# oarodriguez/PhD-QMCLib

Measured on AMD Instinct MI355X. Metric: walker-steps/sec, higher is better.
Workload: dtype f64

## Files before the change

### phd_qmclib_amd/csrc/qmc_device.h

```cpp
#pragma once

#include <hip/hip_runtime.h>
#include <stdint.h>

#include "qmc_math.h"

#define QMC_PI 3.141592653589793238462643383279502884

#define QMC_NSEC 32
#define QMC_SEC_COPIES 1024
#define QMC_NDIAG 4
#if defined(QMC_TIMING)
#define QMC_SECTION(name) qmc_stamp(m, qmc_sec_id(name))
#define QMC_SECTION_PHASE(off) qmc_stamp_phase(off)
#elif defined(QMC_CUTS)
#define QMC_SECTION(name)                                                     \
    do {                                                                      \
        if (m.sec_cut == qmc_sec_id(name) + QMC_SEC_OFF)                      \
            __builtin_amdgcn_endpgm();                                        \
    } while (0)
#define QMC_SECTION_PHASE(off) do { } while (0)
#elif defined(QMC_SECTIONS)
#define QMC_SECTION(name) asm volatile("; SECTION " name)
#define QMC_SECTION_PHASE(off) do { } while (0)
// ... 135 lines not shown
                                                uint32_t stream, double &u0,
                                                double &u1)
{
    uint32_t c[4] = { slot, step, index, stream };
    philox4x32_10(c, (uint32_t)seed, (uint32_t)(seed >> 32));
    u0 = u53(c[0], c[1]);
    u1 = u53(c[2], c[3]);
}

__device__ __forceinline__ void philox2x32_10(uint32_t &c0, uint32_t &c1,
                                              uint32_t k)
{
#pragma unroll
    for (int r = 0; r < 10; ++r) {
        const uint64_t p = (uint64_t)0xD256D193u * c0;
        const uint32_t n0 = (uint32_t)(p >> 32) ^ k ^ c1;
        c1 = (uint32_t)p;
        c0 = n0;
        k += 0x9E3779B9u;
    }
}

__device__ __forceinline__ void vmc_move_block(uint64_t seed, uint32_t slot,
                                               uint32_t step, uint32_t index,
                                               uint32_t &w0, uint32_t &w1)
{
    uint32_t key = (uint32_t)seed ^ ((uint32_t)(seed >> 32) * 0x85EBCA6Bu);
    key += (step >> 26) * 0x632BE5ABu + (slot >> 28) * 0xC2B2AE35u;
    w0 = ((step & 0x3FFFFFFu) << 6) | ((slot >> 22) & 0x3Fu);
    w1 = ((slot & 0x3FFFFFu) << 10) | (index & 0x3FFu);
    philox2x32_10(w0, w1, key);
}

__device__ __forceinline__ double vmc_move_unit(uint32_t w0)
{
    return fma((double)w0, 0x1p-32, 0x1p-33 - 0.5);
}

__device__ __forceinline__ void normal2_from_uniforms(double u0, double u1,
                                                      double &g0, double &g1)
{
    double r = fast_sqrt(fmax(-2.0 * log_pos(1.0 - u0), 1e-300));
    double s, c;
    sincos_halfpi(4.0 * u1, s, c);
    g0 = r * c;
    g1 = r * s;
}

__device__ __forceinline__ void philox_normal2(uint64_t seed, uint32_t slot,
                                               uint32_t step, uint32_t index,
                                               uint32_t stream, double &g0,
                                               double &g1)
{
    double u0, u1;
    philox_uniform2(seed, slot, step, index, stream, u0, u1);
    normal2_from_uniforms(u0, u1, g0, g1);
}

__device__ __forceinline__ void normal2_from_words(uint32_t w0, uint32_t w1,
                                                   double &g0, double &g1)
{
    const double u0 = fma((double)w0, 0x1p-32, 0x1p-33);
    const double u1 = fma((double)w1, 0x1p-32, 0x1p-33);
    const double r = fast_sqrt(-2.0 * log_pos(u0));
    double s, c;
    sincos_halfpi(4.0 * u1, s, c);
    g0 = r * c;
    g1 = r * s;
}

__device__ __forceinline__ void dmc_normal2(uint64_t seed, uint32_t slot,
                                            uint32_t step2, uint32_t index,
                                            double &g0, double &g1)
{
    uint32_t key = (uint32_t)seed ^ ((uint32_t)(seed >> 32) * 0x85EBCA6Bu);
    key += 0x27D4EB2Fu;
    key += (step2 >> 26) * 0x632BE5ABu + (slot >> 28) * 0xC2B2AE35u;
    uint32_t w0 = ((step2 & 0x3FFFFFFu) << 6) | ((slot >> 22) & 0x3Fu);
    uint32_t w1 = ((slot & 0x3FFFFFu) << 10) | (index & 0x3FFu);
    philox2x32_10(w0, w1, key);
    normal2_from_words(w0, w1, g0, g1);
}

__device__ __forceinline__ double wrap_box(double z, double L)
{
    double zw = (z < 0.0) ? z + L : (z >= L) ? z - L : z;
    const bool far = z < -L || z >= 2.0 * L;
    if (__builtin_expect(__ballot(far) != 0ull, 0)) {
        const double r = fma(-L, floor(z / L), z);
        zw = far ? (r < 0.0 ? r + L : r) : zw;
    }
    return zw;
}

template <int G, int P>
struct SlotMap {
    static constexpr bool CONSECUTIVE = (G == 64) && (P >= 2);
};

template <int G, bool PAD>
__device__ __forceinline__ int lanes_in_use(const DevModel &m)
{
    return PAD ? m.ge : G;
}

template <int G, int P, bool PAD>
__device__ __forceinline__ int walker_n(const DevModel &m)
{
    return PAD ? m.n : G * P;
}

template <int G, int P, bool PAD>
__device__ __forceinline__ int lane_particle(const DevModel &m, int gl, int p)
{
    if (SlotMap<G, P>::CONSECUTIVE) return P * gl + p;
    if (!PAD) return gl + G * p;
    const int ge = m.ge;
    return gl < ge ? gl + ge * p : m.n;
}

template <int N>
__device__ __forceinline__ double row_ror_f64(double v)
{
    const int lo = __builtin_amdgcn_update_dpp(0, __double2loint(v), 0x120 + N,
                                               0xf, 0xf, false);
    const int hi = __builtin_amdgcn_update_dpp(0, __double2hiint(v), 0x120 + N,
                                               0xf, 0xf, false);
    return __hiloint2double(hi, lo);
}

template <int G>
__device__ __forceinline__ double group_sum(double v)
{
    static_assert(G >= 16, "lane groups are 16, 32 or 64 lanes");
    v += row_ror_f64<8>(v);
    v += row_ror_f64<4>(v);
    v += row_ror_f64<2>(v);
    v += row_ror_f64<1>(v);
#pragma unroll
    for (int m = 16; m < G; m <<= 1)
        v += __shfl_xor(v, m, 64);
    return v;
}

__device__ __forceinline__ double wave_sum_mfma(double v)
{
    const double r = __builtin_amdgcn_mfma_f64_4x4x4f64(v, 1.0, 0.0, 0, 0, 0);
    double t = __builtin_amdgcn_mfma_f64_4x4x4f64(r, 1.0, 0.0, 0, 0, 0);
    t += row_ror_f64<4>(t);
    t += row_ror_f64<8>(t);
    return t;
}

template <int G, int P>
__device__ __forceinline__ void resort_step(double (&z)[P], int (&lab)[P],
                                            int gl, unsigned parity, int n,
                                            double L, double half_L,
                                            int ge = G)
{
    const int lane = threadIdx.x & 63, base = lane - gl;
    int pg = (parity & 1u) ? ((gl & 1) ? gl + 1 : gl - 1) : (gl ^ 1);
    const bool wrap_hi = pg >= ge, wrap_lo = pg < 0;
    if (wrap_hi) pg = 0;
    if (wrap_lo) pg = ge - 1;
    double z0[P]; int l0[P];
#pragma unroll
    for (int a = 0; a < P; ++a) { z0[a] = z[a]; l0[a] = lab[a]; }
#pragma unroll
    for (int a = 0; a < P; ++a) {
        const int want = wrap_hi ? (a + 1) % P : (wrap_lo ? (a + P - 1) % P : a);
        double zp = 0.0; int lp = 0;
#pragma unroll
        for (int b = 0; b < P; ++b) {
            double zz = __shfl(z0[b], base + pg, 64);
            int ll = __shfl(l0[b], base + pg, 64);
            if (b == want) { zp = zz; lp = ll; }
        }
        const bool valid = gl < ge && (gl + ge * a) < n &&
                           (pg + ge * want) < n;
        const bool lower = wrap_hi ? true : (wrap_lo ? false : gl < pg);
        double d = lower ? zp - z0[a] : z0[a] - zp;
        if (d > half_L) d -= L;
        if (d < -half_L) d += L;
        if (valid && d < 0.0) { z[a] = zp; lab[a] = lp; }
    }
}

template <int G>
__device__ __forceinline__ void resort_linear(double &z, int &lab, int gl,
                                              unsigned parity, int ge)
{
    const int lane = threadIdx.x & 63, base = lane - gl;
    const int pg = (parity & 1u) ? ((gl & 1) ? gl + 1 : gl - 1) : (gl ^ 1);
    const bool has = gl < ge && pg >= 0 && pg < ge;
    const int src = base + (has ? pg : gl);
    const double zp = __shfl(z, src, 64);
    const int lp = __shfl(lab, src, 64);
    const bool take = has && ((gl < pg) ? zp < z : zp > z);
    if (take) { z = zp; lab = lp; }
}

template <int G>
__device__ __forceinline__ int group_ror1_b32(int x)
{
    static_assert(G == 64 || G == 16, "a DPP rotation exists for 16 and 64 lanes");
    if (G == 64) return __builtin_amdgcn_update_dpp(x, x, 0x13C, 0xf, 0xf, false);
    return __builtin_amdgcn_update_dpp(x, x, 0x121, 0xf, 0xf, false);
}
template <int G>
__device__ __forceinline__ double group_ror1(double v)
{
    return __hiloint2double(group_ror1_b32<G>(__double2hiint(v)),
                            group_ror1_b32<G>(__double2loint(v)));
}
template <int G>
__device__ __forceinline__ float group_ror1(float v)
{
    return __int_as_float(group_ror1_b32<G>(__float_as_int(v)));
}

__device__ __forceinline__ double readlane_f64(double v, int lane)
{
    const int lo = __builtin_amdgcn_readlane(__double2loint(v), lane);
    const int hi = __builtin_amdgcn_readlane(__double2hiint(v), lane);
    return __hiloint2double(hi, lo);
}

__device__ __forceinline__ void anchor_seam(double &z, int &lab,
                                            int ge )
{
    const int lane = threadIdx.x & 63;
    const double z0 = readlane_f64(z, 0), zl = readlane_f64(z, ge - 1);
    if (zl < z0) {
        const double z1 = readlane_f64(z, 1), zl1 = readlane_f64(z, ge - 2);
        int src = lane;
        if (zl < z1) {
            if (lane < ge) src = lane == 0 ? ge - 1 : lane - 1;
        } else if (z0 > zl1) {
            if (lane < ge) src = lane == ge - 1 ? 0 : lane + 1;
        }
        z = __shfl(z, src, 64);
        lab = __shfl(lab, src, 64);
    }
}

template <int P>
__device__ __forceinline__ void order_pair(double &za, int &la, double &zb,
                                           int &lb, bool valid)
{
    const bool sw = valid && zb < za;
    const double t = za; const int u = la;
    za = sw ? zb : za; la = sw ? lb : la;
    zb = sw ? t : zb; lb = sw ? u : lb;
}

template <int P>
__device__ __forceinline__ void resort_linear_rows(double (&z)[P], int (&lab)[P],
                                                   int gl, unsigned parity, int n)
{
    static_assert(P % 2 == 0, "consecutive slots: an even number per lane");
    const int i0 = P * gl;
    if (!(parity & 1u)) {
#pragma unroll
        for (int a = 0; a + 1 < P; a += 2)
            order_pair<P>(z[a], lab[a], z[a + 1], lab[a + 1], i0 + a + 1 < n);
    } else {
        const int lane = threadIdx.x & 63;
        const double up = __shfl(z[0], lane + 1, 64);
        const int lup = __shfl(lab[0], lane + 1, 64);
        const double dn = __shfl(z[P - 1], lane - 1, 64);
        const int ldn = __shfl(lab[P - 1], lane - 1, 64);
        const double top = z[P - 1], bot = z[0];
#pragma unroll
        for (int a = 1; a + 1 < P; a += 2)
            order_pair<P>(z[a], lab[a], z[a + 1], lab[a + 1], i0 + a + 1 < n);
        if (gl < 63 && i0 + P < n && up < top) { z[P - 1] = up; lab[P - 1] = lup; }
        if (gl > 0 && i0 < n && dn > bot) { z[0] = dn; lab[0] = ldn; }
    }
}

template <int P, typename T>
__device__ __forceinline__ T row_reg(const T (&v)[P], int r)
{
    T x = v[0];
#pragma unroll
    for (int a = 1; a < P; ++a) x = (r == a) ? v[a] : x;
    return x;
}

template <int P>
__device__ __forceinline__ void anchor_seam_rows(double (&z)[P], int (&lab)[P],
                                                 int n)
{
    const int lane = threadIdx.x & 63;
    const int ln = (n - 1) / P, rn = (n - 1) % P;
    const double z0 = readlane_f64(z[0], 0);
    const double zl = readlane_f64(row_reg<P>(z, rn), ln);
    if (zl < z0) {
        const double z1 = readlane_f64(z[1], 0);
        const int ln2 = (n - 2) / P, rn2 = (n - 2) % P;
        const double zl1 = readlane_f64(row_reg<P>(z, rn2), ln2);
        if (zl < z1) {
            const int labl = __builtin_amdgcn_readlane(row_reg<P>(lab, rn), ln);
            double zin = __shfl(z[P - 1], lane - 1, 64);
            int lin = __shfl(lab[P - 1], lane - 1, 64);
            if (lane == 0) { zin = zl; lin = labl; }
#pragma unroll
            for (int a = P - 1; a >= 1; --a) { z[a] = z[a - 1]; lab[a] = lab[a - 1]; }
// ... 906 lines not shown
```

### phd_qmclib_amd/csrc/qmc_kernels.h

```cpp
#pragma once

#include "qmc_device.h"
#include "qmc_sorted64.h"
#include "qmc_sorted128.h"

static constexpr int BLOCK = 256;

static constexpr int BLOCK64 = 64;
template <int G>
struct WalkBlock {
    static constexpr int N = (G == 64) ? BLOCK64 : BLOCK;
};

template <int GPB>
__device__ __forceinline__ long long walker_of_block(unsigned b, int grp)
{
    if (GPB == 1)
        return ((long long)(b >> 7) << 7) + ((b & 7u) << 4) + ((b & 127u) >> 3);
    return (long long)b * GPB + grp;
}

template <int G, int P, bool PAD, bool ZC, bool DMC = false>
struct StepLds {
    static constexpr int NROWS =
// ... 147 lines not shown
struct alignas(64) VmcRec {
    double wf;
    double ecarry;
    double sum_e, sum_e2;
    long long n_acc;
    long long spare[3];
};
static_assert(sizeof(VmcRec) == 64, "one record = 8 eight-byte words");
typedef unsigned int VmcRecWords __attribute__((ext_vector_type(16)));
#define QMC_CONST __attribute__((address_space(4)))
__device__ __forceinline__ double vmc_rec_word(const VmcRecWords &r, int k)
{
    return __hiloint2double((int)r[2 * k + 1], (int)r[2 * k]);
}

struct VmcArgs {
    double *pos;
    unsigned short *label;
    VmcRec *rec;
    double *ser_wf, *ser_e;
    unsigned char *ser_stat;
    double *ser_pos;
    const double *tape;
    long long tape_steps;
    long long tape_idx;
    long long W;
    long long y;
    unsigned int nsteps;
    int forced;
    int reset_sums;
    int gaussian;
    unsigned int step;
    unsigned int chain0;
    unsigned long long seed;
    double move_spread;
};

template <int G, int P, bool ZC>
struct VmcFused {
    static constexpr bool ON = G == 64 && !ZC && (P == 1 || P == 2);
};

template <int G, int P, bool PAD, bool ZC, bool LEAN, typename R = double,
          bool STEADY = false>
__global__ void __launch_bounds__(WalkBlock<G>::N, lb_waves(G, P, ZC, LB_VMC_P2))
vmc_step_kernel(const DevModel *__restrict__ mp, VmcArgs a)
{
    static_assert(LEAN || !STEADY, "the steady variant is a LEAN kernel");
    const DevModel &m = *mp;
    [[maybe_unused]] constexpr int QMC_SEC_OFF = 0;
    QMC_SECTION("top");
    extern __shared__ double smem[];
    constexpr int GPB = WalkBlock<G>::N / G;
    const int grp = threadIdx.x / G, gl = threadIdx.x % G;
    static_assert(StepLds<G, P, PAD, ZC>::DOUBLES >= GroupLds<G, P, ZC>::DOUBLES,
                  "eval_walker is the fallback on the same LDS region");
    double *lds = smem + (size_t)grp * StepLds<G, P, PAD, ZC>::DOUBLES;
    const long long w = walker_of_block<GPB>(blockIdx.x, grp);
    const bool active = w < a.W;
    if (GPB == 1 && !active) return;
    const long long wr = active ? w : 0;
    const int n = walker_n<G, P, PAD>(m);
    const unsigned int slot = a.chain0 + (unsigned int)wr;
    const bool forced = !STEADY && a.forced != 0;
    const bool reset_sums = !STEADY && a.reset_sums != 0;

    const long long wl = (G == 64) ? qmc_uniform(wr) : wr;
    double wf_cur, e_cur, se = 0.0, se2 = 0.0;
    long long na = 0;
    if constexpr (G == 64) {
        const VmcRecWords r = *(const QMC_CONST VmcRecWords *)(a.rec + wl);
        wf_cur = vmc_rec_word(r, 0);
        e_cur = vmc_rec_word(r, 1);
        se = vmc_rec_word(r, 2);
        se2 = vmc_rec_word(r, 3);
        na = __double_as_longlong(vmc_rec_word(r, 4));
        if (reset_sums) { se = 0.0; se2 = 0.0; na = 0; }
    } else {
        wf_cur = a.rec[wl].wf;
        e_cur = a.rec[wl].ecarry;
    }

    constexpr bool FUSED = STEADY && VmcFused<G, P, ZC>::ON;
    double zc[P];
    int labc[P];
    [[maybe_unused]] double thr = 0.0;
    if constexpr (FUSED) {
#pragma unroll
        for (int p = 0; p < P; ++p) {
            int i = lane_particle<G, P, PAD>(m, gl, p);
            zc[p] = (i < n) ? a.pos[wr * n + i] : 0.0;
            labc[p] = (i < n) ? (int)a.label[wr * n + i] : i;
        }
    }
    bool any_acc = false;
    const unsigned int nst = FUSED ? a.nsteps : 1u;
    bool acc = false;
    [[maybe_unused]] const int gl_top = gl;
    for (unsigned int s = 0; s < nst; ++s) {
    const unsigned int step = a.step + s;
    const int gl = FUSED ? qmc_opaque(gl_top) : gl_top;
    if constexpr (FUSED) {
        if ((s & 63u) == 0u)
            thr = vmc_accept_thresholds(a.seed, slot, step, gl, n);
    }
    QMC_SECTION("load+philox+wrap");
    double zn[P];
    int labn[P];
    double ua = 1.0;
    unsigned int aw0 = 0u, aw1 = 0u;
    bool has0 = false, has1 = false;
    bool outside = false;
#pragma unroll
    for (int p = 0; p < P; ++p) {
        int i = lane_particle<G, P, PAD>(m, gl, p);
        double zp;
        if constexpr (FUSED) {
            zp = zc[p];
            labn[p] = labc[p];
        } else {
            zp = (i < n) ? a.pos[wr * n + i] : 0.0;
            labn[p] = (i < n) ? (int)a.label[wr * n + i] : i;
        }
        const unsigned li = (unsigned)labn[p];
        double d = 0.0;
        if (!forced && i < n) {
            if (!LEAN && a.tape) {
                double tv = a.tape[(wr * a.tape_steps + a.tape_idx) * (n + 1) + li];
                d = a.gaussian ? a.move_spread * tv
                               : (tv - 0.5) * a.move_spread;
            } else if (!LEAN && a.gaussian) {
                double g0, g1;
                philox_normal2(a.seed, slot, step, li, STREAM_VMC_MOVE, g0,
                               g1);
                d = a.move_spread * g0;
            } else {
                uint32_t w0, w1;
                vmc_move_block(a.seed, slot, step, li, w0, w1);
                d = vmc_move_unit(w0) * a.move_spread;
                if constexpr (!FUSED) {
                    if (li == 0u) { aw0 = w1; has0 = true; }
                    if (li == 1u || n == 1) { aw1 = w1; has1 = true; }
                }
            }
        }
        double zs;
        {
#pragma clang fp contract(off)
            zs = zp + d;
        }
        zn[p] = wrap_box(zs, m.L);
        if (forced) outside = outside || zn[p] != zp;
    }
    QMC_SECTION("resort");
    constexpr bool S64 = G == 64 && P == 1 && !ZC;
    constexpr bool S128 = G == 64 && P == 2 && !ZC;
    bool fast = false;
    if (forced)
        outside = __builtin_amdgcn_ballot_w64(outside) != 0ull;
    if constexpr (S64) {
        fast = !m.is_ideal && !outside &&
               sort_lanes64(zn[0], labn[0], gl, PAD ? n : 64) &&
               (PAD ? far_partner_ok_ring(m, zn[0], gl, n)
                    : far_partner_ok64(m, zn[0], gl));
    } else if constexpr (S128) {
        fast = !m.is_ideal && !outside && (!PAD || (n & 1) == 0) &&
               sort_rows128(zn, labn, gl, PAD ? n / 2 : 64) &&
               (PAD ? far_partner_ok_ring128(m, zn, gl, n / 2)
                    : far_partner_ok128(m, zn, gl));
    }
    if constexpr (S64 || S128) {
        if (!fast && !m.is_ideal && gl == 0 && active)
            atomicAdd(m.diag, 1ull);
    } else if constexpr (G == 64 && P == 1) {
        if (!forced) {
            anchor_seam(zn[0], labn[0], n);
            if ((a.step % RESORT_EVERY) == 0)
                resort_linear<G>(zn[0], labn[0], gl,
                                 a.step / RESORT_EVERY, n);
        }
    } else if constexpr (SlotMap<G, P>::CONSECUTIVE) {
        if (!forced) {
            anchor_seam_rows<P>(zn, labn, n);
            if ((a.step % RESORT_EVERY) == 0)
                resort_linear_rows<P>(zn, labn, gl, a.step / RESORT_EVERY, n);
        }
    } else if (!forced && (a.step % RESORT_EVERY) == 0)
        resort_step<G, P>(zn, labn, gl, a.step / RESORT_EVERY, n, m.L,
                          m.half_L, lanes_in_use<G, PAD>(m));
    constexpr bool TWO_PASS = G == 64;
    double F[P], ei[P], e_new = 0.0, wf_new;
    if (S64 && fast) {
        if constexpr (S64)
            eval_sorted64<R, true, false, false, PAD>(
                m, zn[0], gl, lds, F[0], e_new, wf_new);
    } else if (S128 && fast) {
        if constexpr (S128)
            eval_sorted128<R, true, false, false, PAD>(m, zn, gl, lds, F,
                                                       e_new, wf_new);
    } else {
        double z1[P];
#pragma unroll
        for (int p = 0; p < P; ++p) {
            int i = lane_particle<G, P, PAD>(m, gl, p);
            z1[p] = (outside && i < n) ? a.pos[wr * n + i] : zn[p];
        }
        if constexpr (TWO_PASS)
            eval_walker<G, P, PAD, true, false, ZC, R, false, false>(
                m, zn, z1, gl, lds, F, ei, e_new, wf_new);
        else
            eval_walker<G, P, PAD, true, false, ZC, R>(m, zn, z1, gl, lds, F,
                                                       ei, e_new, wf_new);
    }
    QMC_SECTION("metropolis+store");
    if (FUSED) {
    } else if (!forced) {
        if (!LEAN && a.tape) {
            ua = a.tape[(wr * a.tape_steps + a.tape_idx) * (n + 1) + n];
        } else if (!LEAN && a.gaussian) {
            double u1;
            philox_uniform2(a.seed, slot, step, 0u, STREAM_VMC_ACCEPT, ua,
                            u1);
        } else {
            const unsigned long long bal0 = __ballot(has0);
            const unsigned long long bal1 = __ballot(has1);
            unsigned int hi, lo;
            if (G == 64) {
                const int src0 = __builtin_amdgcn_readfirstlane(
                    (int)__ffsll((long long)bal0) - 1) & 63;
                const int src1 = __builtin_amdgcn_readfirstlane(
                    (int)__ffsll((long long)bal1) - 1) & 63;
                hi = (unsigned)__builtin_amdgcn_readlane((int)aw0, src0);
                lo = (unsigned)__builtin_amdgcn_readlane((int)aw1, src1);
            } else {
// ... 52 lines not shown
            for (int p = 0; p < P; ++p) {
                zc[p] = zn[p];
                labc[p] = labn[p];
            }
            any_acc = true;
        } else {
#pragma unroll
            for (int p = 0; p < P; ++p) {
                int i = lane_particle<G, P, PAD>(m, gl, p);
                if (i < n && !forced) {
                    a.pos[w * n + i] = zn[p];
                    a.label[w * n + i] = (unsigned short)labn[p];
                }
            }
        }
        if (!FUSED) {
            wf_cur = wf_new;
            e_cur = e_new;
        }
    }
    if constexpr (FUSED) {
        if (acc) {
            wf_cur = qmc_uniform_f64(wf_new);
            const double e2 = qmc_lane_f64(e_new, 2);
            const double e3 = qmc_lane_f64(e_new, 3);
            e_cur = qmc_lane_f64(e_new, 1);
            se = se + e2;
            se2 = fma(e3, e3, se2);
            na = na + 1;
        } else {
            se = se + e_cur;
            se2 = fma(e_cur, e_cur, se2);
        }
        se = qmc_uniform_f64(se);
        se2 = qmc_uniform_f64(se2);
        continue;
    }
    if (!LEAN && a.ser_pos) {
#pragma unroll
        for (int p = 0; p < P; ++p) {
            int i = lane_particle<G, P, PAD>(m, gl, p);
            if (i < n) {
                const bool moved = acc && !forced;
                const int lb = moved ? labn[p] : (int)a.label[w * n + i];
                a.ser_pos[(a.y * a.W + w) * n + lb] =
                    moved ? zn[p] : a.pos[w * n + i];
            }
        }
    }
    if (G == 64) {
        const double sum1 = se + e_cur;
        const double sum2 = fma(e_cur, e_cur, se2);
        const long long na1 = qmc_uniform(na + (acc ? 1 : 0));
        double v = __longlong_as_double((gl == 4) ? na1 : 0ll);
        v = (gl == 0) ? wf_cur : v;
        v = (gl == 1) ? e_cur : v;
        v = (gl == 2) ? sum1 : v;
        v = (gl == 3) ? sum2 : v;
        if (gl < 8) reinterpret_cast<double *>(a.rec + wl)[gl] = v;
    }
    if (gl == 0) {
        if (G != 64) {
            VmcRec *r = a.rec + w;
            if (!reset_sums) { se = r->sum_e; se2 = r->sum_e2; na = r->n_acc; }
            r->wf = wf_cur;
            r->ecarry = e_cur;
            r->sum_e = se + e_cur;
            r->sum_e2 = fma(e_cur, e_cur, se2);
            r->n_acc = na + (acc ? 1 : 0);
        }
        if (!LEAN) {
            if (a.ser_wf) a.ser_wf[a.y * a.W + w] = wf_cur;
            if (a.ser_e) a.ser_e[a.y * a.W + w] = e_cur;
            if (a.ser_stat) a.ser_stat[a.y * a.W + w] = acc ? 1 : 0;
        }
    }
    }
    if constexpr (FUSED) {
        QMC_SECTION("fused_store");
        if (any_acc) {
#pragma unroll
            for (int p = 0; p < P; ++p) {
                int i = lane_particle<G, P, PAD>(m, gl, p);
                if (i < n) {
                    a.pos[w * n + i] = zc[p];
                    a.label[w * n + i] = (unsigned short)labc[p];
                }
            }
        }
        double v = __longlong_as_double((gl == 4) ? qmc_uniform(na) : 0ll);
        v = (gl == 0) ? wf_cur : v;
        v = (gl == 1) ? e_cur : v;
        v = (gl == 2) ? se : v;
        v = (gl == 3) ? se2 : v;
        if (gl < 8) reinterpret_cast<double *>(a.rec + wl)[gl] = v;
    }
    QMC_SECTION("end");
}

struct DmcCtl {
    long long prev_nw;
    long long nw;
    double ref_energy;
    double total_energy, total_weight;
    double e_t, w_t;
    long long spare_nw;
    unsigned int step;
    unsigned int pad;
};

struct EvolveArgs {
    const double *ppos, *pdrift, *penergy;
    double *cpos, *cdrift, *cenergy, *cweight;
    const unsigned short *plabel;
    unsigned short *clabel;
    double *eslot;
    const long long *ref;
    const DmcCtl *ctl;
    const double *g_tape;
    double *spare;
    long long maxw;
    double dt, sigma;
    unsigned long long seed;
    unsigned int slot0;
    int fix_stale;
};

template <int G, int P, bool PAD, bool ZC, typename R = double>
__global__ void __launch_bounds__(WalkBlock<G>::N, lb_waves(G, P, ZC, LB_DMC_P2))
dmc_evolve_kernel(const DevModel *__restrict__ mp, EvolveArgs a)
{
    const DevModel &m = *mp;
    [[maybe_unused]] constexpr int QMC_SEC_OFF = 0;
    extern __shared__ double smem[];
    constexpr int GPB = WalkBlock<G>::N / G;
    const int grp = threadIdx.x / G, gl = threadIdx.x % G;
    static_assert(StepLds<G, P, PAD, ZC, true>::DOUBLES >=
                      GroupLds<G, P, ZC>::DOUBLES,
                  "eval_walker is the fallback on the same LDS region");
    double *lds = smem + (size_t)grp * StepLds<G, P, PAD, ZC, true>::DOUBLES;
    const long long s = walker_of_block<GPB>(blockIdx.x, grp);
    const long long nw = a.ctl->nw;
    if ((GPB == 1 ? s : (long long)blockIdx.x * GPB) >= nw) return;
    QMC_SECTION("top");
    const bool active = s < nw;
    const long long sr = active ? s : 0;
    const int n = walker_n<G, P, PAD>(m);
    const unsigned int step = a.ctl->step;
    const double ref_energy = a.ctl->ref_energy;
    const long long spare_nw = a.ctl->spare_nw;
    const long long su = (G == 64) ? qmc_uniform(sr) : sr;
    const long long par = a.ref[su];
    double e_par = 0.0, e_slot = 0.0;
    if (G == 64) {
        e_par = a.penergy[par];
        e_slot = a.eslot[su];
    }

    QMC_SECTION("load+philox+wrap");
    double z[P];
    int lab[P];
#pragma unroll
    for (int p = 0; p < P; ++p) {
        int i = lane_particle<G, P, PAD>(m, gl, p);
        double zz = 0.0;
        lab[p] = i;
        if (i < n) {
// ... 88 lines not shown
```

### phd_qmclib_amd/csrc/qmc_sorted128.h

```cpp
#pragma once

#include "qmc_sorted64.h"

template <typename R> struct SlotPair;
template <> struct SlotPair<double> {
    typedef double type __attribute__((ext_vector_type(2)));
};
template <> struct SlotPair<float> {
    typedef float type __attribute__((ext_vector_type(2)));
};
template <typename R>
__device__ __forceinline__ typename SlotPair<R>::type ld_pair(const R *p)
{
    return *(const typename SlotPair<R>::type *)p;
}

__device__ __forceinline__ bool rows_ascending128(const double (&z)[2],
                                                  int nl = 64)
{
    const int lo = __double2loint(z[0]), hi = __double2hiint(z[0]);
    const double up = __hiloint2double(
        __builtin_amdgcn_update_dpp(0, hi, 0x130, 0xf, 0xf, true),
        __builtin_amdgcn_update_dpp(0, lo, 0x130, 0xf, 0xf, true));
    const int lane = threadIdx.x & 63;
    const bool bad = (lane < nl) &
                     ((z[1] < z[0]) | ((lane < nl - 1) & (up < z[1])));
    return __builtin_amdgcn_ballot_w64(bad) == 0ull;
}

__device__ __forceinline__ bool sort_rows128(double (&z)[2], int (&lab)[2], int gl,
                                             int nl = 64)
{
    if (rows_ascending128(z, nl)) return true;
    const int lane = threadIdx.x & 63;
    const int a_up = (lane >= nl - 1 ? lane : lane + 1) << 2;
    const int a_dn = (lane == 0 || lane >= nl ? lane : lane - 1) << 2;
    for (int it = 0; it < 66; ++it) {
        anchor_seam_rows<2>(z, lab, 2 * nl);
        {
            const bool sw = lane < nl && z[1] < z[0];
            const double t = z[0]; const int u = lab[0];
            z[0] = sw ? z[1] : z[0]; lab[0] = sw ? lab[1] : lab[0];
            z[1] = sw ? t : z[1];    lab[1] = sw ? u : lab[1];
        }
        {
            const double up = __hiloint2double(
                __builtin_amdgcn_ds_bpermute(a_up, __double2hiint(z[0])),
                __builtin_amdgcn_ds_bpermute(a_up, __double2loint(z[0])));
            const int lup = __builtin_amdgcn_ds_bpermute(a_up, lab[0]);
            const double dn = __hiloint2double(
                __builtin_amdgcn_ds_bpermute(a_dn, __double2hiint(z[1])),
                __builtin_amdgcn_ds_bpermute(a_dn, __double2loint(z[1])));
            const int ldn = __builtin_amdgcn_ds_bpermute(a_dn, lab[1]);
            const bool t_up = lane < nl - 1 && up < z[1];
            const bool t_dn = lane > 0 && lane < nl && dn > z[0];
            z[1] = t_up ? up : z[1]; lab[1] = t_up ? lup : lab[1];
            z[0] = t_dn ? dn : z[0]; lab[0] = t_dn ? ldn : lab[0];
        }
        if (rows_ascending128(z, nl)) return true;
    }
    return false;
}

__device__ __forceinline__ bool far_partner_ok128(const DevModel &m,
                                                  const double (&z)[2], int gl)
{
    const double zp = __shfl_xor(z[0], 32, 64);
    const double d = (gl < 32) ? (z[1] - zp) + m.L : z[1] - zp;
    return __builtin_amdgcn_ballot_w64(d >= m.L_minus_rm) == 0ull;
}

__device__ __forceinline__ bool far_partner_ok_ring128(const DevModel &m,
                                                       const double (&z)[2],
                                                       int gl, int nl)
{
    const bool live = gl < nl;
    int src = gl - nl / 2;
    const bool wrapped = src < 0;
    if (wrapped) src += nl;
    const double zp = __shfl(z[0], live ? src : gl, 64);
    const double d = wrapped ? (z[1] - zp) + m.L : z[1] - zp;
    return __builtin_amdgcn_ballot_w64(live & (d >= m.L_minus_rm)) == 0ull;
}

template <typename R, bool WF, bool EN, bool REUSE, bool PAD = false>
__device__ __forceinline__ void eval_sorted128(const DevModel &m,
                                               const double (&z)[2], int gl,
                                               double *lds, double (&F)[2],
                                               double &E, double &logwf)
{
    constexpr int G = 64, NS = 128, H = SortedRows<NS>::H,
                  ROW = SortedRows<NS>::ROW;
    constexpr bool COT = SortedCot<WF, EN, REUSE>::ON;
    constexpr bool TAN = SortedCot<WF, EN, REUSE>::TAN;
    typedef SortedCot<WF, EN, REUSE> RowsOf;
    R *lS = (R *)lds, *lC = lS + ROW, *lSU = lS + RowsOf::ROW_SU * ROW,
      *lCU = lS + 3 * ROW, *lZ = lS + RowsOf::ROW_Z * ROW;
    const int n = PAD ? m.n : NS;
    const int nl = n / 2;
    const int K = nl / 2;
    const bool half_last = !PAD || (nl & 1) == 0;
    const int kfull = half_last ? K - 1 : K;
    const bool live = !PAD || gl < nl;
    const unsigned long long live_mask =
        PAD ? __builtin_amdgcn_ballot_w64(live) : ~0ull;
    [[maybe_unused]] constexpr int QMC_SEC_OFF = REUSE ? QMC_NSEC / 2 : 0;
    QMC_SECTION("tables+onebody");
    Own64<R> o[2];
    SortedOneBody ob[2];
    PTab ta[2];
    SortedPub pub[2];
#pragma unroll
    for (int a = 0; a < 2; ++a)
        sorted_particle_setup<R, WF, EN, REUSE, NS, false>(
            m, z[a], 2 * gl + a, (R *)lds, o[a], ob[a], n, ta[a], pub[a]);
#define QMC_S128_ST(row, i, v0, v1)                                           \
        *(typename SlotPair<R>::type *)((row) + (i)) =                        \
            typename SlotPair<R>::type{ (R)(v0), (R)(v1) }
    if (!REUSE && live) {
        const int up = H + 2 * gl, lo = up - n;
        QMC_S128_ST(lS, up, pub[0].s, pub[1].s);
        if (!COT) QMC_S128_ST(lC, up, pub[0].c, pub[1].c);
        QMC_S128_ST(lSU, up, pub[0].su, pub[1].su);
        if (!TAN) QMC_S128_ST(lCU, up, pub[0].cu, pub[1].cu);
        QMC_S128_ST(lZ, up, z[0], z[1]);
        if (lo >= 2) {
            if (COT) {
                QMC_S128_ST(lS, lo, pub[0].s, pub[1].s);
            } else {
                QMC_S128_ST(lS, lo, -pub[0].s, -pub[1].s);
                QMC_S128_ST(lC, lo, -pub[0].c, -pub[1].c);
            }
            QMC_S128_ST(lSU, lo, pub[0].su_lo, pub[1].su_lo);
            if (!TAN) QMC_S128_ST(lCU, lo, pub[0].cu_lo, pub[1].cu_lo);
            QMC_S128_ST(lZ, lo, z[0] - m.L, z[1] - m.L);
        }
    } else if (REUSE && COT && live) {
        const int up = H + 2 * gl, lo = up - n;
        QMC_S128_ST(lS, up, pub[0].s, pub[1].s);
        if (TAN) QMC_S128_ST(lSU, up, pub[0].su, pub[1].su);
        if (lo >= 2) {
            QMC_S128_ST(lS, lo, pub[0].s, pub[1].s);
            if (TAN) QMC_S128_ST(lSU, lo, pub[0].su_lo, pub[1].su_lo);
        }
    }
#undef QMC_S128_ST
    if (!REUSE || COT) {
        __builtin_amdgcn_fence(__ATOMIC_RELEASE, "wavefront");
        __builtin_amdgcn_wave_barrier();
        __builtin_amdgcn_fence(__ATOMIC_ACQUIRE, "wavefront");
    }
    int nb_wave = 0;
// ... 161 lines not shown
                if (h00) { asm volatile(""); Qs = q_fma(q00, q00, Qs); }      \
                if (h10) { asm volatile(""); Qs = q_fma(q10, q10, Qs); }      \
                if (h01) { asm volatile(""); Qs = q_fma(q01, q01, Qs); }      \
                if (h11) { asm volatile(""); Qs = q_fma(q11, q11, Qs); }      \
            }                                                                 \
        }                                                                     \
    }
#define QMC_S128_LONG_XY(oa, cs, cc, X, Y)                                    \
    const R Y = COT ? (cs) - (oa).s : (oa).s * (cc) - (oa).c * (cs);          \
    R X = 0;                                                                  \
    if (EN) X = COT ? q_fma((oa).s, (cs), (R)1)                               \
                    : (oa).c * (cc) + (oa).s * (cs);
#define QMC_S128_LONG_STEP(s0_, c0_, s1_, c1_)                                \
    {                                                                         \
        QMC_S128_LONG_XY(o[0], s0_, c0_, X00, Y00)                            \
        QMC_S128_LONG_XY(o[1], s0_, c0_, X10, Y10)                            \
        QMC_S128_LONG_XY(o[0], s1_, c1_, X01, Y01)                            \
        QMC_S128_LONG_XY(o[1], s1_, c1_, X11, Y11)                            \
        if (WF && live) PL *= (Y00 * Y10) * (Y01 * Y11);                      \
        if (EN) {                                                             \
            const R q00 = pair_div(X00, Y00), q10 = pair_div(X10, Y10);       \
            const R q01 = pair_div(X01, Y01), q11 = pair_div(X11, Y11);       \
            Fr[0] += q00 + q01;                                               \
            Fr[1] += q10 + q11;                                               \
            T[0] -= q00 + q10;                                                \
            T[1] -= q01 + q11;                                                \
            T[0] = (R)QMC_S128_ROR(T[0]);                                     \
            T[1] = (R)QMC_S128_ROR(T[1]);                                     \
            Qall = q_fma(q00, q00, Qall); Qall = q_fma(q10, q10, Qall);       \
            Qall = q_fma(q01, q01, Qall); Qall = q_fma(q11, q11, Qall);       \
        }                                                                     \
    }
    {
        typedef typename SlotPair<R>::type R2;
        R2 as = ld_pair(pS - 2 * k), ac = ld_pair(pC - 2 * k);
        R2 bs = ld_pair(pS - 2 * (k + 1)), bc = ld_pair(pC - 2 * (k + 1));
        const R zt0 = o[0].zt;
#pragma clang loop unroll(disable)
        while (k < kfull) {
            if (__builtin_amdgcn_ballot_w64(live & (pZ[-2 * k + 1] > zt0)) ==
                0ull)
                break;
            QMC_S128_STEP(as[0], ac[0], as[1], ac[1], k, false)
            as = ld_pair(pS - 2 * (k + 2)); ac = ld_pair(pC - 2 * (k + 2));
            QMC_S128_STEP(bs[0], bc[0], bs[1], bc[1], k + 1, false)
            bs = ld_pair(pS - 2 * (k + 3)); bc = ld_pair(pC - 2 * (k + 3));
            k += 2;
            if (WF) {
                q_fold(PS, eS);
                q_fold(PL, eL);
            }
        }
        QMC_SECTION("rotation");
#pragma clang loop unroll(disable)
        while (k < kfull) {
            QMC_S128_LONG_STEP(as[0], ac[0], as[1], ac[1])
            as = ld_pair(pS - 2 * (k + 2)); ac = ld_pair(pC - 2 * (k + 2));
            QMC_S128_LONG_STEP(bs[0], bc[0], bs[1], bc[1])
            bs = ld_pair(pS - 2 * (k + 3)); bc = ld_pair(pC - 2 * (k + 3));
            k += 2;
            if (WF) q_fold(PL, eL);
        }
        if (k <= kfull) {
            QMC_S128_STEP(as[0], ac[0], as[1], ac[1], k, false)
            ++k;
            as = bs; ac = bc;
        }
        QMC_SECTION("rotation_last_step");
        if (half_last) QMC_S128_STEP(as[0], ac[0], as[1], ac[1], k, true)
    }
#undef QMC_S128_STEP
#undef QMC_S128_LONG_STEP
#undef QMC_S128_LONG_XY
#undef QMC_S128_XY
#undef QMC_S128_SHORT_XY
    if (EN) {
        if (PAD) {
            int src = gl + kfull + 1;
            if (src >= nl) src -= nl;
            src = live ? src : gl;
            Fr[0] += __shfl(T[0], src, 64);
            Fr[1] += __shfl(T[1], src, 64);
        } else {
            Fr[0] += __shfl_xor(T[0], G / 2, 64);
            Fr[1] += __shfl_xor(T[1], G / 2, 64);
        }
    }
#undef QMC_S128_ROR
#undef QMC_S128_ALL

    QMC_SECTION("energy+logwf");
    double e_lane = 0.0, e_consts = 0.0;
    if (EN) {
        F[0] = fma(m.a_long, (double)Fr[0], ob[0].ldz);
        F[1] = fma(m.a_long, (double)Fr[1], ob[1].ldz);
        const double Qall_d = (double)Qall, Qs_d = (double)Qs;
        const double pk = (Qs_d + (Qall_d - Qs_d) * m.inv_beta) * m.a_long_sq;
        e_lane = fma(2.0, pk, kin1_sum) - F[0] * F[0] - F[1] * F[1];
        if (PAD && !live) e_lane = 0.0;
        if (nb_counted)
            e_consts += (double)(n - nb_wave) * m.e0 +
                        (double)nb_wave * (m.v_barrier - m.v0_minus_e0);
        const int nlong = n * (n - 1) / 2 - ns;
        e_consts += 2.0 * (m.k2sq * (double)ns + m.b_long * (double)nlong);
    }
    double lw = 0.0;
    if (WF) {
        const double LN2 = 0.693147180559945309417;
        q_fold(PS, eS);
        q_fold(PL, eL);
        const double PS_d = (double)PS, PL_d = (double)PL;
        if (!m.is_free && m.ob_table) {
            const double lSv = log_pos(PS_d);
            lw = fma(m.beta, log_pos(PL_d) - lSv, lSv);
        } else {
            lw = log_pos(ob[0].prod1 * ob[1].prod1 * PS_d) +
                 m.beta * log_pos(fast_div(PL_d, PS_d));
        }
        lw += LN2 * ((double)eS + m.beta * (double)(eL - eS));
        lw -= ob[0].xoff + ob[1].xoff;
        if (PAD && !live) lw = 0.0;
    }
    if (EN) E = group_sum<G>(e_lane) + e_consts;
    if (WF) logwf = group_sum<G>(lw);
}
```

### phd_qmclib_amd/csrc/qmc_sorted64.h

```cpp
#pragma once

#include "qmc_device.h"


template <bool WF, bool EN, bool REUSE>
struct SortedCot {
    static constexpr bool ON = EN && !WF;
    static constexpr bool TAN = ON;
    static constexpr bool COMPACT = TAN && !REUSE;
    static constexpr int ROW_SU = COMPACT ? 1 : 2;
    static constexpr int ROW_Z = COMPACT ? 2 : 4;
    static constexpr int ROWS = COMPACT ? 3 : 5;
};

__device__ __forceinline__ double div_clamped(double x, double y, double tiny)
{
    const double ya = fmax(__builtin_fabs(y), tiny);
    return fast_div(x, __builtin_copysign(ya, y));
}

__device__ __forceinline__ double wave_shr1_f64(double v)
{
    const int lo = __double2loint(v), hi = __double2hiint(v);
    return __hiloint2double(
        __builtin_amdgcn_update_dpp(0, hi, 0x138, 0xf, 0xf, true),
        __builtin_amdgcn_update_dpp(0, lo, 0x138, 0xf, 0xf, true));
}

__device__ __forceinline__ unsigned long long lanes_inverted64(double z,
                                                               int nl = 64)
{
    const bool live = (int)(threadIdx.x & 63) < nl;
    return __builtin_amdgcn_ballot_w64(live & (z < wave_shr1_f64(z)));
}

__device__ __forceinline__ bool lanes_ascending64(double z, int nl = 64)
{
    return lanes_inverted64(z, nl) == 0ull;
}

__device__ __forceinline__ void cmpxchg_pass64(double &z, int &lab, int addr,
                                               int flip)
{
    const int plo = __builtin_amdgcn_ds_bpermute(addr, __double2loint(z));
    const int phi = __builtin_amdgcn_ds_bpermute(addr, __double2hiint(z));
    const int pl = __builtin_amdgcn_ds_bpermute(addr, lab);
    const double zp = __hiloint2double(phi, plo);
    const double d = zp - z;
    const bool take = __hiloint2double(__double2hiint(d) ^ flip,
                                       __double2loint(d)) < 0.0;
    z = take ? zp : z;
    lab = take ? pl : lab;
}

__device__ __forceinline__ bool sort_lanes64(double &z, int &lab, int gl,
                                             int nl = 64)
{
    unsigned long long inv = lanes_inverted64(z, nl);
    if (inv == 0ull) return true;
    const int odd = gl & 1;
    const int pe = gl ^ 1;
    const int addr_even = ((gl >= nl || pe >= nl) ? gl : pe) << 2;
    const int po = odd ? (gl + 1) : (gl - 1);
    const int addr_odd = ((gl >= nl || po < 0 || po >= nl) ? gl : po) << 2;
    const int flip_even = odd << 31;
    const int flip_odd = (odd ^ 1) << 31;
    const unsigned long long ends = 2ull | (1ull << (nl - 1));
    for (int it = 0; it < 140; ++it) {
        if (inv & ends) anchor_seam(z, lab, nl);
        if (inv & 0xAAAAAAAAAAAAAAAAull)
            cmpxchg_pass64(z, lab, addr_even, flip_even);
        if (inv & 0x5555555555555555ull)
            cmpxchg_pass64(z, lab, addr_odd, flip_odd);
        inv = lanes_inverted64(z, nl);
        if (inv == 0ull) return true;
    }
    return false;
}

__device__ __forceinline__ bool far_partner_ok64(const DevModel &m, double z,
                                                 int gl)
{
    const double zp = __shfl_xor(z, 32, 64);
    const double d = (gl < 32) ? (z - zp) + m.L : z - zp;
    return __builtin_amdgcn_ballot_w64(d >= m.L_minus_rm) == 0ull;
}

__device__ __forceinline__ bool far_partner_ok_ring(const DevModel &m, double z,
                                                    int gl, int nl)
{
    const int K = nl / 2;
    const bool live = gl < nl;
    int src = gl - K;
    const bool wrapped = src < 0;
    if (wrapped) src += nl;
    const double zp = __shfl(z, live ? src : gl, 64);
    const double d = wrapped ? (z - zp) + m.L : z - zp;
    return __builtin_amdgcn_ballot_w64(live & (d >= m.L_minus_rm)) == 0ull;
}

template <typename R>
struct Own64 {
    R s, c;
    R s0, c0;
    R ks0, kc0;
    R zt;
};

struct SortedOneBody {
    double ldz = 0.0;
    double kin1 = 0.0;
    double xoff = 0.0;
    double prod1 = 1.0;
    bool barrier = false;
};

template <int NS>
struct SortedRows {
    static constexpr int H = NS / 2 + (NS > 64 ? 2 : 1);
    static constexpr int ROW = NS + H;
    static_assert(NS <= 64 || (H % 2 == 0 && ROW % 2 == 0),
                  "two slots per lane: 16-byte aligned pairs");
};

struct SortedPub {
    double s, c, su, cu, su_lo, cu_lo;
};

template <typename R, bool WF, bool EN, bool REUSE, int NS, bool WRITE = true>
__device__ __forceinline__ void sorted_particle_setup(const DevModel &m, double z,
                                                      int slot, R *tab,
                                                      Own64<R> &o,
                                                      SortedOneBody &ob,
                                                      int n, PTab &ta,
                                                      SortedPub &pub)
{
    constexpr int H = SortedRows<NS>::H, ROW = SortedRows<NS>::ROW;
    typedef SortedCot<WF, EN, REUSE> RowsOf;
    R *lS = tab, *lC = lS + ROW, *lSU = lS + RowsOf::ROW_SU * ROW,
      *lCU = lS + 3 * ROW, *lZ = lS + RowsOf::ROW_Z * ROW;
    TrigRow trow;
    const bool trig_ok = !REUSE && m.trig_table && trig_tab_load(m, z, trow);
    if (!m.is_free && m.ob_table) {
        double lf = 0.0;
        one_body_tab<WF, EN>(m, z, ob.ldz, lf, ob.barrier);
        if (WF) ob.xoff = -lf;
        if (EN) {
            if (m.uniform_barrier)
                ob.kin1 = ob.ldz * ob.ldz;
            else
                ob.kin1 = fma(ob.ldz, ob.ldz,
                              one_body_kin_const(m, z, ob.barrier));
        }
    } else if (!m.is_free) {
        double kp, f1, xo;
        one_body(m, z, ob.ldz, kp, f1, xo);
        if (EN) ob.kin1 = kp;
        if (WF) { ob.prod1 = f1; ob.xoff = xo; }
    }
    __builtin_amdgcn_sched_barrier(0);
    if (REUSE) {
        ta.s = (double)lS[H + slot]; ta.c = (double)lC[H + slot];
        ta.su = (double)lSU[H + slot]; ta.cu = (double)lCU[H + slot];
    } else if (trig_ok) {
        trig_tab_finish(m, trow, ta);
    } else {
        sincos_halfpi(z * m.two_over_L, ta.s, ta.c);
        sincos_halfpi(z * m.k2_2pi, ta.su, ta.cu);
// ... 200 lines not shown
    if (WF && mine) PL *= Y;
#define QMC_S64_TALLY(q, sh, mine)                                            \
    if (mine) {                                                               \
        Qall = q_fma(q, q, Qall);                                             \
        if (sh) {                                                             \
            asm volatile("");                                                 \
            Qs = q_fma(q, q, Qs);                                             \
        }                                                                     \
    }
    R as_ = pS[-k], ac_ = pC[-k];
    R bs_ = pS[-(k + 1)], bc_ = pC[-(k + 1)];
#pragma clang loop unroll(disable)
    while (k < kfull) {
        QMC_S64_XY(as_, ac_, k, false, Xa, Ya, sha, minea)
        as_ = pS[-(k + 2)]; ac_ = pC[-(k + 2)];
        QMC_S64_XY(bs_, bc_, k + 1, false, Xb, Yb, shb, mineb)
        bs_ = pS[-(k + 3)]; bc_ = pC[-(k + 3)];
        k += 2;
        if (EN) {
            const R qa = pair_div(Xa, Ya), qb = pair_div(Xb, Yb);
            QMC_S64_ADD_Q(qa, k - 2)
            QMC_S64_ADD_Q(qb, k - 1)
            QMC_S64_TALLY(qa, sha, minea)
            QMC_S64_TALLY(qb, shb, mineb)
        }
        if (WF && sizeof(R) == 4) {
            q_fold(PS, eS);
            q_fold(PL, eL);
        }
        if (shb_m == 0ull) break;
    }
    QMC_SECTION("rotation");
#define QMC_S64_LONG(cs, cc)                                                  \
    {                                                                         \
        const R Y = COT ? (cs) - o.s : o.s * (cc) - o.c * (cs);               \
        if (WF && live) PL *= Y;                                              \
        if (EN) {                                                             \
            const R X = COT ? q_fma(o.s, (cs), (R)1)                          \
                            : o.c * (cc) + o.s * (cs);                        \
            const R q = pair_div(X, Y);                                       \
            QMC_S64_ADD_Q(q, k)                                               \
            if (live) Qall = q_fma(q, q, Qall);                               \
        }                                                                     \
        ++k;                                                                  \
    }
#pragma clang loop unroll(disable)
    while (k < kfull) {
        QMC_S64_LONG(pS[-k], pC[-k])
        QMC_S64_LONG(pS[-k], pC[-k])
        if (WF && sizeof(R) == 4) q_fold(PL, eL);
    }
    as_ = pS[-k]; ac_ = pC[-k];
    bs_ = pS[-(k + 1)]; bc_ = pC[-(k + 1)];
#undef QMC_S64_LONG
    if (k <= kfull) {
        QMC_S64_XY(as_, ac_, k, false, Xa, Ya, sha, minea)
        if (EN) {
            const R q = pair_div(Xa, Ya);
            QMC_S64_ADD_Q(q, k)
            QMC_S64_TALLY(q, sha, minea)
        }
        ++k;
        as_ = bs_; ac_ = bc_;
    }
    QMC_SECTION("rotation_last_step");
    if (half_last) {
        QMC_S64_XY(as_, ac_, k, true, Xl, Yl, shl, minel)
        if (EN) {
            const R q = pair_div(Xl, Yl);
            Fr += q;
            QMC_S64_TALLY(q, shl, minel)
        }
    }
#undef QMC_S64_XY
#undef QMC_S64_TALLY
#undef QMC_S64_ADD_Q
#undef QMC_S64_ALL
    if (EN) {
        if (PAD) {
            int src = gl + kfull + 1;
            if (src >= nl) src -= nl;
            Fr += __shfl(T, live ? src : gl, 64);
        } else {
            Fr += __shfl_xor(T, G / 2, 64);
        }
    }
#undef QMC_S64_ROR

    QMC_SECTION("energy+logwf");
    double e_lane = 0.0, e_consts = 0.0;
    if (EN) {
        F = fma(m.a_long, (double)Fr, ldz);
        const double Qall_d = (double)Qall, Qs_d = (double)Qs;
        const double pk = (Qs_d + (Qall_d - Qs_d) * m.inv_beta) * m.a_long_sq;
        e_lane = fma(2.0, pk, kin1) - F * F;
        if (PAD && !live) e_lane = 0.0;
        if (nb_counted)
            e_consts += (double)(nl - nb_wave) * m.e0 +
                        (double)nb_wave * (m.v_barrier - m.v0_minus_e0);
        const int nlong = nl * (nl - 1) / 2 - ns;
        e_consts += 2.0 * (m.k2sq * (double)ns + m.b_long * (double)nlong);
    }
    double lw = 0.0;
    if (WF) {
        const double LN2 = 0.693147180559945309417;
        const double PS_d = (double)PS, PL_d = (double)PL;
        if (sizeof(R) == 8 && !m.is_free && m.ob_table) {
            const bool odd = gl & 1;
            double own = odd ? PS_d : PL_d, give = odd ? PL_d : PS_d;
            if (PAD && !live) { own = 1.0; give = 1.0; }
            const double got = __hiloint2double(
                __builtin_amdgcn_update_dpp(0, __double2hiint(give), 0xB1, 0xf,
                                            0xf, false),
                __builtin_amdgcn_update_dpp(0, __double2loint(give), 0xB1, 0xf,
                                            0xf, false));
            int bh = __double2hiint(m.beta), bl = __double2loint(m.beta);
            int oh = __double2hiint(m.one_minus_beta),
                ol = __double2loint(m.one_minus_beta);
            asm volatile("" : "+s"(bh), "+s"(bl), "+s"(oh), "+s"(ol));
            lw = __hiloint2double(odd ? oh : bh, odd ? ol : bl) *
                 log_pos(own * got);
            if (PAD && gl >= ((nl + 1) & ~1)) lw = 0.0;
            if (!PAD || live) lw -= xoff;
        } else if (!m.is_free && m.ob_table) {
            const double lSv = log_pos(PS_d);
            lw = fma(m.beta, log_pos(PL_d) - lSv, lSv);
        } else {
            lw = log_pos(prod1 * PS_d) +
                 m.beta * log_pos(fast_div(PL_d, PS_d));
        }
        const bool merged = sizeof(R) == 8 && !m.is_free && m.ob_table;
        if (sizeof(R) == 4)
            lw += LN2 * ((double)eS + m.beta * (double)(eL - eS));
        if (!merged) {
            lw -= xoff;
            if (PAD && !live) lw = 0.0;
        }
    }
    if (WF && EN) {
        E = wave_sum_mfma(e_lane);
        logwf = wave_sum_mfma(lw);
        E += e_consts;
    } else if (EN) {
        E = wave_sum_mfma(e_lane) + e_consts;
    } else {
        logwf = wave_sum_mfma(lw);
    }
}
```

Before: 781.2 million.

## Use permlane32_swap and SGPR-mask selects for cross-half exchanges and branches

Replaces the __shfl_xor(…,32) cross-half exchanges in the sorted64/sorted128 paths with the permlane32_swap intrinsic, which avoids an LDS bpermute round trip. Per-lane conditional selects (wrap, compare-exchange, odd/even lane choice) become v_cndmask driven by ballot masks or constant lane masks held in SGPRs. In the fused, non-padded path the i<n guards are dropped at compile time. This trims VALU and LDS work from the inner step, but inline asm may limit compiler scheduling, and the constant odd-lane mask assumes the particle-to-lane layout maps gl parity to lane parity.

After: 785.8 million (median of 6 runs). No clear change (+0.6%).

```diff
diff --git a/phd_qmclib_amd/csrc/qmc_device.h b/phd_qmclib_amd/csrc/qmc_device.h
--- a/phd_qmclib_amd/csrc/qmc_device.h
+++ b/phd_qmclib_amd/csrc/qmc_device.h
@@ -241,9 +241,33 @@
     normal2_from_words(w0, w1, g0, g1);
 }
 
+__device__ __forceinline__ int qmc_sel_i32(unsigned long long mask, int a, int b)
+{
+    int r;
+    asm("v_cndmask_b32_e64 %0, %1, %2, %3" : "=v"(r) : "v"(b), "v"(a), "s"(mask));
+    return r;
+}
+__device__ __forceinline__ double qmc_sel_f64(unsigned long long mask, double a,
+                                              double b)
+{
+    return __hiloint2double(
+        qmc_sel_i32(mask, __double2hiint(a), __double2hiint(b)),
+        qmc_sel_i32(mask, __double2loint(a), __double2loint(b)));
+}
+#define QMC_LANES_ODD 0xAAAAAAAAAAAAAAAAull
+#define QMC_LANES_LOWER 0x00000000FFFFFFFFull
+
+template <bool SMASK = false>
 __device__ __forceinline__ double wrap_box(double z, double L)
 {
-    double zw = (z < 0.0) ? z + L : (z >= L) ? z - L : z;
+    double zw;
+    if constexpr (SMASK) {
+        const unsigned long long below = __builtin_amdgcn_ballot_w64(z < 0.0);
+        const unsigned long long above = __builtin_amdgcn_ballot_w64(z >= L);
+        zw = qmc_sel_f64(below, z + L, qmc_sel_f64(above, z - L, z));
+    } else {
+        zw = (z < 0.0) ? z + L : (z >= L) ? z - L : z;
+    }
     const bool far = z < -L || z >= 2.0 * L;
     if (__builtin_expect(__ballot(far) != 0ull, 0)) {
         const double r = fma(-L, floor(z / L), z);
@@ -383,6 +407,38 @@
     const int lo = __builtin_amdgcn_readlane(__double2loint(v), lane);
     const int hi = __builtin_amdgcn_readlane(__double2hiint(v), lane);
     return __hiloint2double(hi, lo);
+}
+
+__device__ __forceinline__ void wave_halves32_f64(double v, double &lower,
+                                                  double &upper)
+{
+    const unsigned lo = (unsigned)__double2loint(v),
+                   hi = (unsigned)__double2hiint(v);
+    const auto rl = __builtin_amdgcn_permlane32_swap(lo, lo, false, false);
+    const auto rh = __builtin_amdgcn_permlane32_swap(hi, hi, false, false);
+    lower = __hiloint2double((int)rh[0], (int)rl[0]);
+    upper = __hiloint2double((int)rh[1], (int)rl[1]);
+}
+__device__ __forceinline__ double wave_swap32_f64(double v)
+{
+    double lower, upper;
+    wave_halves32_f64(v, lower, upper);
+    return qmc_sel_f64(QMC_LANES_LOWER, upper, lower);
+}
+__device__ __forceinline__ float wave_swap32_f32(float v)
+{
+    const unsigned x = (unsigned)__float_as_int(v);
+    const auto r = __builtin_amdgcn_permlane32_swap(x, x, false, false);
+    return __int_as_float(qmc_sel_i32(QMC_LANES_LOWER, (int)r[1], (int)r[0]));
+}
+
+__device__ __forceinline__ double wave_swap32(double v)
+{
+    return wave_swap32_f64(v);
+}
+__device__ __forceinline__ float wave_swap32(float v)
+{
+    return wave_swap32_f32(v);
 }
 
 __device__ __forceinline__ void anchor_seam(double &z, int &lab,
diff --git a/phd_qmclib_amd/csrc/qmc_kernels.h b/phd_qmclib_amd/csrc/qmc_kernels.h
--- a/phd_qmclib_amd/csrc/qmc_kernels.h
+++ b/phd_qmclib_amd/csrc/qmc_kernels.h
@@ -253,6 +253,7 @@
     }
 
     constexpr bool FUSED = STEADY && VmcFused<G, P, ZC>::ON;
+    constexpr bool FULL = FUSED && !PAD;
     double zc[P];
     int labc[P];
     [[maybe_unused]] double thr = 0.0;
@@ -260,8 +261,8 @@
 #pragma unroll
         for (int p = 0; p < P; ++p) {
             int i = lane_particle<G, P, PAD>(m, gl, p);
-            zc[p] = (i < n) ? a.pos[wr * n + i] : 0.0;
-            labc[p] = (i < n) ? (int)a.label[wr * n + i] : i;
+            zc[p] = (FULL || i < n) ? a.pos[wr * n + i] : 0.0;
+            labc[p] = (FULL || i < n) ? (int)a.label[wr * n + i] : i;
         }
     }
     bool any_acc = false;
@@ -295,7 +296,7 @@
         }
         const unsigned li = (unsigned)labn[p];
         double d = 0.0;
-        if (!forced && i < n) {
+        if (!forced && (FULL || i < n)) {
             if (!LEAN && a.tape) {
                 double tv = a.tape[(wr * a.tape_steps + a.tape_idx) * (n + 1) + li];
                 d = a.gaussian ? a.move_spread * tv
@@ -320,7 +321,7 @@
 #pragma clang fp contract(off)
             zs = zp + d;
         }
-        zn[p] = wrap_box(zs, m.L);
+        zn[p] = wrap_box<FUSED>(zs, m.L);
         if (forced) outside = outside || zn[p] != zp;
     }
     QMC_SECTION("resort");
@@ -539,7 +540,7 @@
 #pragma unroll
             for (int p = 0; p < P; ++p) {
                 int i = lane_particle<G, P, PAD>(m, gl, p);
-                if (i < n) {
+                if (FULL || i < n) {
                     a.pos[w * n + i] = zc[p];
                     a.label[w * n + i] = (unsigned short)labc[p];
                 }
diff --git a/phd_qmclib_amd/csrc/qmc_sorted128.h b/phd_qmclib_amd/csrc/qmc_sorted128.h
--- a/phd_qmclib_amd/csrc/qmc_sorted128.h
+++ b/phd_qmclib_amd/csrc/qmc_sorted128.h
@@ -65,9 +65,14 @@
 __device__ __forceinline__ bool far_partner_ok128(const DevModel &m,
                                                   const double (&z)[2], int gl)
 {
-    const double zp = __shfl_xor(z[0], 32, 64);
-    const double d = (gl < 32) ? (z[1] - zp) + m.L : z[1] - zp;
-    return __builtin_amdgcn_ballot_w64(d >= m.L_minus_rm) == 0ull;
+    double z0l, z0u;
+    wave_halves32_f64(z[0], z0l, z0u);
+    const unsigned long long far_lower =
+        __builtin_amdgcn_ballot_w64((z[1] - z0u) + m.L >= m.L_minus_rm);
+    const unsigned long long far_upper =
+        __builtin_amdgcn_ballot_w64(z[1] - z0l >= m.L_minus_rm);
+    return ((far_lower & QMC_LANES_LOWER) | (far_upper & ~QMC_LANES_LOWER)) ==
+           0ull;
 }
 
 __device__ __forceinline__ bool far_partner_ok_ring128(const DevModel &m,
@@ -395,8 +400,8 @@
             Fr[0] += __shfl(T[0], src, 64);
             Fr[1] += __shfl(T[1], src, 64);
         } else {
-            Fr[0] += __shfl_xor(T[0], G / 2, 64);
-            Fr[1] += __shfl_xor(T[1], G / 2, 64);
+            Fr[0] += wave_swap32(T[0]);
+            Fr[1] += wave_swap32(T[1]);
         }
     }
 #undef QMC_S128_ROR
diff --git a/phd_qmclib_amd/csrc/qmc_sorted64.h b/phd_qmclib_amd/csrc/qmc_sorted64.h
--- a/phd_qmclib_amd/csrc/qmc_sorted64.h
+++ b/phd_qmclib_amd/csrc/qmc_sorted64.h
@@ -47,10 +47,10 @@
     const int pl = __builtin_amdgcn_ds_bpermute(addr, lab);
     const double zp = __hiloint2double(phi, plo);
     const double d = zp - z;
-    const bool take = __hiloint2double(__double2hiint(d) ^ flip,
-                                       __double2loint(d)) < 0.0;
-    z = take ? zp : z;
-    lab = take ? pl : lab;
+    const unsigned long long take = __builtin_amdgcn_ballot_w64(
+        __hiloint2double(__double2hiint(d) ^ flip, __double2loint(d)) < 0.0);
+    z = qmc_sel_f64(take, zp, z);
+    lab = qmc_sel_i32(take, pl, lab);
 }
 
 __device__ __forceinline__ bool sort_lanes64(double &z, int &lab, int gl,
@@ -81,9 +81,11 @@
 __device__ __forceinline__ bool far_partner_ok64(const DevModel &m, double z,
                                                  int gl)
 {
-    const double zp = __shfl_xor(z, 32, 64);
-    const double d = (gl < 32) ? (z - zp) + m.L : z - zp;
-    return __builtin_amdgcn_ballot_w64(d >= m.L_minus_rm) == 0ull;
+    double zl, zu;
+    wave_halves32_f64(z, zl, zu);
+    const double e = zl - zu;
+    return __builtin_amdgcn_ballot_w64((e + m.L >= m.L_minus_rm) |
+                                       (-e >= m.L_minus_rm)) == 0ull;
 }
 
 __device__ __forceinline__ bool far_partner_ok_ring(const DevModel &m, double z,
@@ -450,7 +452,7 @@
             if (src >= nl) src -= nl;
             Fr += __shfl(T, live ? src : gl, 64);
         } else {
-            Fr += __shfl_xor(T, G / 2, 64);
+            Fr += wave_swap32(T);
         }
     }
 #undef QMC_S64_ROR
@@ -474,8 +476,8 @@
         const double LN2 = 0.693147180559945309417;
         const double PS_d = (double)PS, PL_d = (double)PL;
         if (sizeof(R) == 8 && !m.is_free && m.ob_table) {
-            const bool odd = gl & 1;
-            double own = odd ? PS_d : PL_d, give = odd ? PL_d : PS_d;
+            double own = qmc_sel_f64(QMC_LANES_ODD, PS_d, PL_d),
+                   give = qmc_sel_f64(QMC_LANES_ODD, PL_d, PS_d);
             if (PAD && !live) { own = 1.0; give = 1.0; }
             const double got = __hiloint2double(
                 __builtin_amdgcn_update_dpp(0, __double2hiint(give), 0xB1, 0xf,
@@ -486,7 +488,8 @@
             int oh = __double2hiint(m.one_minus_beta),
                 ol = __double2loint(m.one_minus_beta);
             asm volatile("" : "+s"(bh), "+s"(bl), "+s"(oh), "+s"(ol));
-            lw = __hiloint2double(odd ? oh : bh, odd ? ol : bl) *
+            lw = __hiloint2double(qmc_sel_i32(QMC_LANES_ODD, oh, bh),
+                                  qmc_sel_i32(QMC_LANES_ODD, ol, bl)) *
                  log_pos(own * got);
             if (PAD && gl >= ((nl + 1) & ~1)) lw = 0.0;
             if (!PAD || live) lw -= xoff;
```
